# tbuckworth/train-procgen-pytorch

Hardware: AMD Instinct MI355X
Metric: env steps/sec (whole node), coinrun hard-500 IMPALA-CNN PPO (higher is better)
Workload: dtype bf16

## Files before the change

### train-procgen-pytorch_amd/csrc/device_util.h

```cpp
#pragma once
#include <hip/hip_runtime.h>
#include <stdint.h>

typedef short bf16x8 __attribute__((ext_vector_type(8)));
typedef short s16x4 __attribute__((ext_vector_type(4)));
typedef s16x4 __attribute__((address_space(3))) * lds_s16x4_ptr;
#define MFMA16(a, b, c) __builtin_amdgcn_mfma_f32_16x16x4f32((a), (b), (c), 0, 0, 0)
#define MFMA_BF16(a, b, c) __builtin_amdgcn_mfma_f32_16x16x32_bf16((a), (b), (c), 0, 0, 0)

template <typename T>
__device__ __forceinline__ T wave_sum(T v) {
#pragma unroll
    for (int o = 32; o > 0; o >>= 1) v += __shfl_down(v, o, 64);
    return v;
}
__device__ __forceinline__ float wave_max(float v) {
#pragma unroll
    for (int o = 32; o > 0; o >>= 1) v = fmaxf(v, __shfl_down(v, o, 64));
    return v;
}
template <typename T>
__device__ __forceinline__ T block_sum256(T v, T* sbuf) {
    v = wave_sum(v);
    const int lane = threadIdx.x & 63, w = threadIdx.x >> 6;
// ... 48 lines not shown
#pragma unroll
    for (int j = 0; j < 2; ++j)
        lo[j] = __builtin_amdgcn_perm(__builtin_amdgcn_perm((unsigned)best[4 * j + 3], (unsigned)best[4 * j + 2], 0x0c0c0400u),
                                      __builtin_amdgcn_perm((unsigned)best[4 * j + 1], (unsigned)best[4 * j], 0x0c0c0400u), 0x05040100u);
    val = (uint4){mi_keys_to_bf16x2(kv[0]), mi_keys_to_bf16x2(kv[1]), mi_keys_to_bf16x2(kv[2]), mi_keys_to_bf16x2(kv[3])};
    arg = (uint2){0x08080808u - lo[0], 0x08080808u - lo[1]};
}
__device__ __forceinline__ unsigned mi_relu_bf16x2(unsigned w) {
    return __builtin_bit_cast(unsigned, __builtin_elementwise_max(__builtin_bit_cast(mi_s16x2, w), (mi_s16x2){0, 0}));
}
__device__ __forceinline__ float mi_bf16x4_lane(uint2 w, int r) {
    const unsigned u = (r >> 1) ? w.y : w.x;
    return (r & 1) ? bfw_hi(u) : bfw_lo(u);
}
__device__ __forceinline__ uint2 mi_pk_bf16x4(const float (&v)[4]) { return (uint2){mi_pk_bf16(v[0], v[1]), mi_pk_bf16(v[2], v[3])}; }
```

### train-procgen-pytorch_amd/csrc/resblock_bf16.hip

```cpp
#include "common.h"
#include "device_util.h"
#include <hip/hip_ext.h>
#include <mutex>
#include <type_traits>

__device__ __forceinline__ bool rb_pos(uint2 w, int r) {
    const unsigned u = (r >> 1) ? w.y : w.x;
    return (r & 1) ? (int)u >= 0x10000 : (short)(unsigned short)u > (short)0;
}

#ifndef RB_ROWPAD8
#define RB_ROWPAD8 1
#endif
#ifndef RB_SWZ16
#define RB_SWZ16 1
#endif
#ifndef RB_S32
#define RB_S32 48
#endif
template <int C_, int HW_, int TH_, int NIMG_, int NT_ = 256>
struct RbCfg {
    static constexpr int C = C_, HW = HW_, TH = TH_, NIMG = NIMG_, NT = NT_, NW = NT_ / 64;
    static constexpr bool WHOLE = (TH == HW);
    static_assert(WHOLE || NIMG == 1, "row tiles hold one image");
// ... 384 lines not shown
    static constexpr size_t LDS_BYTES = (size_t)5 * T_ELEMS * 2;
    static_assert(LDS_BYTES <= 160 * 1024 && NMT % 8 == 0 && NPX * 4 % 256 == 0, "one workgroup per CU; tile pairs per wave; whole staging words");
    static __device__ __forceinline__ int org(int pl) { return (pl / (HW * HW)) * IMG_ELEMS + (((pl / HW) % HW) * P + pl % HW) * S; }
};
template <class C>
__global__ __launch_bounds__(512, 2) void resblock_pair32r_bf16_kernel(ResblockPairArgs a) {
    extern __shared__ __attribute__((aligned(16))) unsigned short smem_h[];
    unsigned short* s_x = smem_h;
    unsigned short* s_a1 = s_x + C::T_ELEMS;
    unsigned short* s_h = s_a1 + C::T_ELEMS;
    unsigned short* s_a2 = s_h + 2 * C::T_ELEMS;
    const int tid = threadIdx.x, lane = tid & 63, i = lane & 15, kq = lane >> 4;
    const int wv = __builtin_amdgcn_readfirstlane(tid >> 6);
    const bool role_a = wv < 4;
    const int rw = wv & 3;
    for (int e = tid; e < 5 * C::T_ELEMS / 8; e += 512) ((uint4*)smem_h)[e] = (uint4){0u, 0u, 0u, 0u};
    f32x4 st[36];
    f32x4 bq[2][2];
    {
        const unsigned short* bk1 = a.bank[role_a ? 0 : 2];
        const unsigned short* bk2 = a.bank[role_a ? 1 : 3];
        const float* b1 = a.b[role_a ? 0 : 2];
        const float* b2 = a.b[role_a ? 1 : 3];
#pragma unroll
        for (int m = 0; m < 9; ++m)
#pragma unroll
            for (int nb = 0; nb < 2; ++nb) {
                st[2 * m + nb] = __builtin_bit_cast(f32x4, *(const uint4*)(bk1 + (nb * 16 + i) * C::WS + m * 32 + kq * 8));
                st[18 + 2 * m + nb] = __builtin_bit_cast(f32x4, *(const uint4*)(bk2 + (nb * 16 + i) * C::WS + m * 32 + kq * 8));
            }
#pragma unroll
        for (int nb = 0; nb < 2; ++nb) { bq[0][nb] = *(const f32x4*)(b1 + nb * 16 + kq * 4); bq[1][nb] = *(const f32x4*)(b2 + nb * 16 + kq * 4); }
    }
    __builtin_amdgcn_s_waitcnt(0x0F70);
    auto koffc = [](int m) { return ((m / 3) * C::P + (m % 3)) * C::S; };
    constexpr int CENTER = (C::P + 1) * C::S;
    const int nitem = (a.n + C::NIMG - 1) / C::NIMG;
    const int nimg = ((int)blockIdx.x < nitem) ? (nitem - 1 - (int)blockIdx.x) / (int)gridDim.x + 1 : 0;
    typedef unsigned rp_u32x4 __attribute__((ext_vector_type(4)));
    rp_u32x4 rx[C::NWORD];
    auto load = [&](int k) {
        const long long it = blockIdx.x + (long long)(k < nimg ? k : nimg - 1) * gridDim.x;
#pragma unroll
        for (int q = 0; q < C::NWORD; ++q) {
            if constexpr (C::NIMG == 1) rx[q] = *(const rp_u32x4*)(a.x + it * (C::HW * C::HW * C::C) + (size_t)(tid + q * 256) * 8);
            else {
                const int e = tid + q * 256, pl = e >> 2;
                long long n = it * C::NIMG + pl / (C::HW * C::HW); n = n < a.n ? n : a.n - 1;
                rx[q] = *(const rp_u32x4*)(a.x + (n * (C::HW * C::HW) + pl % (C::HW * C::HW)) * C::C + (e & 3) * 8);
            }
        }
    };
    auto conv_tiles = [&](const unsigned short* s_src, const int (&org)[2], const int b0, bool relu, f32x4 (&acc)[2][2]) {
        bf16x8 av[2][5];
        auto rd = [&](int q, int m) {
            bf16x8 v = *(const bf16x8*)(s_src + org[q] + kq * 8 + koffc(m));
            if (relu) { const uint4 u = __builtin_bit_cast(uint4, v); v = __builtin_bit_cast(bf16x8, (uint4){mi_relu_bf16x2(u.x), mi_relu_bf16x2(u.y), mi_relu_bf16x2(u.z), mi_relu_bf16x2(u.w)}); }
            return v;
        };
#pragma unroll
// ... 15 lines not shown
    if (role_a && nimg > 0) load(0);
    for (int step = 0; step <= nimg; ++step) {
        const bool on = role_a ? step < nimg : step >= 1;
        const int k = role_a ? step : step - 1;
        const long long item0 = (blockIdx.x + (long long)(k < 0 ? 0 : k) * gridDim.x) * C::NIMG;
        const long long base = item0 * (C::HW * C::HW * C::C);
        const int left = a.n - (int)item0;
        unsigned short* s_in = role_a ? s_x : s_h + ((step - 1) & 1) * C::T_ELEMS;
        unsigned short* s_mid = role_a ? s_a1 : s_a2;
        unsigned short* a_out = role_a ? a.a1_out : a.a2_out;
        unsigned short* y_out = role_a ? a.y1_out : a.y2_out;
        __syncthreads();
        if (role_a && on) {
#pragma unroll
            for (int q = 0; q < C::NWORD; ++q) {
                const int e = tid + q * 256, pl = e >> 2;
                *(rp_u32x4*)(s_x + C::org(pl) + CENTER + (e & 3) * 8) = rx[q];
            }
            load(step + 1);
        }
        __syncthreads();
        if (on) {
            for (int t = rw; t < C::NMT; t += 8) {
                int pl[2], org[2];
#pragma unroll
                for (int q2 = 0; q2 < 2; ++q2) { pl[q2] = (t + 4 * q2) * 16 + i; org[q2] = C::org(pl[q2]); }
                f32x4 acc[2][2];
                conv_tiles(s_in, org, 0, true, acc);
#pragma unroll
                for (int q2 = 0; q2 < 2; ++q2)
#pragma unroll
                    for (int nb = 0; nb < 2; ++nb) {
                        float v[4];
#pragma unroll
                        for (int r = 0; r < 4; ++r) v[r] = acc[q2][nb][r] + bq[0][nb][r];
                        const uint2 raw = mi_pk_bf16x4(v);
                        if (a_out && (C::NIMG == 1 || pl[q2] / (C::HW * C::HW) < left)) *(uint2*)(a_out + base + (long long)pl[q2] * C::C + nb * 16 + kq * 4) = raw;
                        *(uint2*)(s_mid + org[q2] + CENTER + nb * 16 + kq * 4) = (uint2){mi_relu_bf16x2(raw.x), mi_relu_bf16x2(raw.y)};
                    }
            }
        }
        __syncthreads();
        if (on) {
            unsigned short* s_nxt = s_h + (step & 1) * C::T_ELEMS;
            for (int t = rw; t < C::NMT; t += 8) {
                int pl[2], org[2];
                uint2 sk[2][2];
#pragma unroll
                for (int q2 = 0; q2 < 2; ++q2) {
                    pl[q2] = (t + 4 * q2) * 16 + i; org[q2] = C::org(pl[q2]);
                    sk[q2][0] = *(const uint2*)(s_in + org[q2] + CENTER + kq * 4); sk[q2][1] = *(const uint2*)(s_in + org[q2] + CENTER + 16 + kq * 4);
                }
                f32x4 acc[2][2];
                conv_tiles(s_mid, org, 18, false, acc);
#pragma unroll
                for (int q2 = 0; q2 < 2; ++q2)
#pragma unroll
                    for (int nb = 0; nb < 2; ++nb) {
                        float v[4];
#pragma unroll
                        for (int r = 0; r < 4; ++r) v[r] = acc[q2][nb][r] + bq[1][nb][r] + mi_bf16x4_lane(sk[q2][nb], r);
                        const uint2 raw = mi_pk_bf16x4(v);
                        if (y_out && (C::NIMG == 1 || pl[q2] / (C::HW * C::HW) < left)) *(uint2*)(y_out + base + (long long)pl[q2] * C::C + nb * 16 + kq * 4) = raw;
                        if (role_a) *(uint2*)(s_nxt + org[q2] + CENTER + nb * 16 + kq * 4) = raw;
                    }
            }
        }
    }
}
template <class C>
static void launch_rbp32r(const ResblockPairArgs& a, hipStream_t st) {
    static std::once_flag attr;
    std::call_once(attr, [] { hipFuncSetAttribute((const void*)resblock_pair32r_bf16_kernel<C>, hipFuncAttributeMaxDynamicSharedMemorySize, (int)C::LDS_BYTES); });
    const int items = (a.n + C::NIMG - 1) / C::NIMG, grid = items > 256 ? 256 : items;
    if (grid < 1) return;
    hipLaunchKernelGGL(resblock_pair32r_bf16_kernel<C>, dim3(grid), dim3(512), C::LDS_BYTES, st, a);
}
using RBR_32_16 = RbPair32R<16, 1>;

template <class C>
// ... 289 lines not shown
                                   const unsigned short* bank2_t, const unsigned short* bank1_t, float* slab2, float* slab1, hipStream_t st, hipEvent_t done_ev) {
    const int grid = resblock_bwd_full_grid(n);
    if (grid < 1) return;
    RbFullArgs a{(const unsigned short*)dy, (const unsigned short*)a_fwd, (const unsigned short*)x_fwd, (unsigned short*)dx_out, (unsigned short*)da_out,
                 bank2_t, bank1_t, slab2, slab1, n};
    constexpr size_t LDS_D = RBFULL16D_NBUF * RbFull16S::TILE_BYTES > RbFull16S::RED_BYTES ? RBFULL16D_NBUF * RbFull16S::TILE_BYTES : RbFull16S::RED_BYTES;
    static_assert(LDS_D > 80 * 1024 && LDS_D <= 160 * 1024, "one workgroup per CU");
    static std::once_flag attr;
    std::call_once(attr, [] { hipFuncSetAttribute((const void*)resblock_bwd_full16d_bf16_kernel, hipFuncAttributeMaxDynamicSharedMemorySize, (int)LDS_D); });
    if (done_ev) hipExtLaunchKernelGGL(resblock_bwd_full16d_bf16_kernel, dim3(grid), dim3(512), (unsigned)LDS_D, st, nullptr, done_ev, 0, a);
    else hipLaunchKernelGGL(resblock_bwd_full16d_bf16_kernel, dim3(grid), dim3(512), LDS_D, st, a);
}

template <int HW_, int NT_, int TH_>
struct RbFull32T {
    static constexpr int C = 32, HW = HW_, TH = TH_, S = RB_S32, P = HW + 2, TPI = HW / TH, NT = NT_;
    static constexpr int XR = TH + 4, YR = TH + 2;
    static constexpr int X_ELEMS = XR * P * S, Y_ELEMS = YR * P * S;
    static constexpr int NK = 9, WS = NK * 32 + 16;
    static constexpr int NMT1 = YR * HW / 16, NMT2 = TH * HW / 16;
    static constexpr int NX = XR * HW * 4, NA = YR * HW * 4;
    static constexpr int NSTEP = TH * HW / 32;
    static constexpr int NQ = 18;
    static constexpr int WLEN = C * 9 * C, SLAB = WLEN + C;
};
#ifndef RB32S_TH
#define RB32S_TH 16
#endif
using RbFull32W = RbFull32T<16, 512, RB32S_TH>;
#ifdef WG_TIMING
__device__ unsigned long long g_rb_timing[8];
#define RTCK(k) do { if ((tid & 255) == 0) { const long long now_ = clock64(); tacc_[k] += now_ - tlast_; tlast_ = now_; } } while (0)
#else
#define RTCK(k) do { } while (0)
#endif
template <class C>
__global__ __launch_bounds__(512, 2) void resblock_bwd_full32s_bf16_kernel(RbFullArgs a) {
    static_assert(C::NT == 512 && C::HW == 16, "16x16 images, 8 waves");
    extern __shared__ __attribute__((aligned(16))) unsigned short smem_h[];
    unsigned short* s_x = smem_h;
    unsigned short* s_y = s_x + C::X_ELEMS;
    unsigned short* s_a = s_y + C::Y_ELEMS;
    unsigned short* s_p = s_a + C::Y_ELEMS;
    const int tid = threadIdx.x, lane = tid & 63, wave = tid >> 6, i = lane & 15, kq = lane >> 4, rq = (lane & 15) >> 2, cp = lane & 3;
    const int wv = __builtin_amdgcn_readfirstlane(wave);
    const bool conv_role = wv < 4;
#ifdef WG_TIMING
    long long tacc_[4] = {0, 0, 0, 0}, tlast_ = clock64();
#endif
    const int rw = wv & 3;
    for (int e = tid; e < (C::X_ELEMS + 3 * C::Y_ELEMS) / 8; e += C::NT) ((uint4*)smem_h)[e] = (uint4){0u, 0u, 0u, 0u};
    constexpr bool WHOLE = C::TPI == 1;
    constexpr int NT2 = 256, NIN = C::HW * C::HW * 4;
    constexpr int KX2 = WHOLE ? NIN / NT2 : (C::NX + NT2 - 1) / NT2, KA2 = WHOLE ? NIN / NT2 : (C::NA + NT2 - 1) / NT2;
    static_assert(!WHOLE || NIN % NT2 == 0, "whole words per staging thread");
    constexpr int NST = (22 + KX2 + 2 * KA2) > 36 ? (22 + KX2 + 2 * KA2) : 36;
    f32x4 st[NST];
    constexpr int QM = 5;
    const int qcnt = (C::NQ - rw + 3) / 4;
    if (conv_role) {
#pragma unroll
        for (int m = 0; m < 9; ++m)
#pragma unroll
            for (int nb = 0; nb < 2; ++nb) {
                st[2 * m + nb] = __builtin_bit_cast(f32x4, *(const uint4*)(a.bank2_t + (nb * 16 + i) * C::WS + m * 32 + kq * 8));
                st[18 + 2 * m + nb] = __builtin_bit_cast(f32x4, *(const uint4*)(a.bank1_t + (nb * 16 + i) * C::WS + m * 32 + kq * 8));
            }
    } else {
#pragma unroll
        for (int q = 0; q < NST; ++q) st[q] = (f32x4){0.f, 0.f, 0.f, 0.f};
    }
    __builtin_amdgcn_s_waitcnt(0x0F70);
    const bf16x8 ones = __builtin_bit_cast(bf16x8, (uint4){0x3f803f80u, 0x3f803f80u, 0x3f803f80u, 0x3f803f80u});
    auto koffc = [](int m) { return ((m / 3) * C::P + (m % 3)) * C::S; };

    const int nwork = a.n * C::TPI;
    const int t2 = tid - 256;
    auto load = [&](int work) {
        const long long img = work / C::TPI; const int ty0 = (work % C::TPI) * C::TH;
        if constexpr (WHOLE) {
            const long long o = img * (C::HW * C::HW * C::C) + t2 * 8;
#pragma unroll
            for (int k = 0; k < KX2; ++k) {
                st[22 + k] = __builtin_bit_cast(f32x4, *(const uint4*)(a.dy + o + k * NT2 * 8));
                st[22 + KX2 + k] = __builtin_bit_cast(f32x4, *(const uint4*)(a.a_fwd + o + k * NT2 * 8));
                st[22 + KX2 + KA2 + k] = __builtin_bit_cast(f32x4, *(const uint4*)(a.x_fwd + o + k * NT2 * 8));
            }
            return;
        }
#pragma unroll
        for (int k = 0; k < KX2; ++k) {
            const int e = t2 + k * NT2;
            uint4 v = {0u, 0u, 0u, 0u};
            if (e < C::NX) { const int c8 = e & 3, px = (e >> 2) % C::HW, gy = ty0 - 2 + e / (4 * C::HW);
                             if (gy >= 0 && gy < C::HW) v = *(const uint4*)(a.dy + ((img * C::HW + gy) * C::HW + px) * C::C + c8 * 8); }
            st[22 + k] = __builtin_bit_cast(f32x4, v);
        }
#pragma unroll
        for (int k = 0; k < KA2; ++k) {
            const int e = t2 + k * NT2;
            uint4 va = {0u, 0u, 0u, 0u}, vp = {0u, 0u, 0u, 0u};
            if (e < C::NA) { const int c8 = e & 3, px = (e >> 2) % C::HW, gy = ty0 - 1 + e / (4 * C::HW);
                             if (gy >= 0 && gy < C::HW) { const long long o = ((img * C::HW + gy) * C::HW + px) * C::C + c8 * 8;
                                                          va = *(const uint4*)(a.a_fwd + o); vp = *(const uint4*)(a.x_fwd + o); } }
            st[22 + KX2 + k] = __builtin_bit_cast(f32x4, va); st[22 + KX2 + KA2 + k] = __builtin_bit_cast(f32x4, vp);
        }
    };
    const int orow0 = ((kq >> 1) * C::P + 4 * (kq & 1) + rq) * C::S + 4 * cp;
    struct WgBase { int d, b[QM]; };
    auto wg_bases = [&](const unsigned short* s_d, int d_off, const unsigned short* s_src) {
        WgBase w;
        w.d = (int)(s_d - smem_h) + orow0 + d_off;
#pragma unroll
        for (int qq = 0; qq < QM; ++qq) {
            const int q = rw + 4 * (qq < 4 ? qq : (qcnt > 4 ? 4 : 0)), tap = q >> 1, ib = q & 1;
            w.b[qq] = (int)(s_src - smem_h) + orow0 + ((tap / 3) * C::P + (tap % 3)) * C::S + ib * 16;
            asm volatile("" : "+v"(w.b[qq]));
        }
        asm volatile("" : "+v"(w.d));
        return w;
// ... 10 lines not shown
        for (int cb = 0; cb < 2; ++cb) d[cb] = tr(w.d, cb * 16);
#pragma unroll
        for (int qq = 0; qq < QM; ++qq) b[qq] = tr(w.b[qq], 0);
        asm volatile("" ::: "memory");
        if (bias) { st[20] = MFMA_BF16(d[0], ones, st[20]); st[21] = MFMA_BF16(d[1], ones, st[21]); }
#pragma unroll
        for (int qq = 0; qq < QM; ++qq)
            if (qq < qcnt) {
#pragma unroll
                for (int cb = 0; cb < 2; ++cb) st[a0 + 2 * qq + cb] = MFMA_BF16(d[cb], b[qq], st[a0 + 2 * qq + cb]);
            }
    };

    if (!conv_role && (int)blockIdx.x < nwork) load(blockIdx.x);
    for (int work = blockIdx.x; work < nwork; work += gridDim.x) {
        const long long img = work / C::TPI; const int ty0 = (work % C::TPI) * C::TH;
        __syncthreads();
        RTCK(3);
        if (!conv_role && WHOLE) {
            const int o = ((t2 >> 6) * C::P + ((t2 >> 2) & (C::HW - 1)) + 1) * C::S + (t2 & 3) * 8;
#pragma unroll
            for (int k = 0; k < KX2; ++k) {
                const int ok = o + k * (NT2 / 64) * C::P * C::S;
                const uint4 va = __builtin_bit_cast(uint4, st[22 + KX2 + k]), vp = __builtin_bit_cast(uint4, st[22 + KX2 + KA2 + k]);
                *(uint4*)(s_x + ok + 2 * C::P * C::S) = __builtin_bit_cast(uint4, st[22 + k]);
                *(uint4*)(s_a + ok + C::P * C::S) = (uint4){mi_relu_bf16x2(va.x), mi_relu_bf16x2(va.y), mi_relu_bf16x2(va.z), mi_relu_bf16x2(va.w)};
                *(uint4*)(s_p + ok + C::P * C::S) = (uint4){mi_relu_bf16x2(vp.x), mi_relu_bf16x2(vp.y), mi_relu_bf16x2(vp.z), mi_relu_bf16x2(vp.w)};
            }
        } else if (!conv_role) {
#pragma unroll
            for (int k = 0; k < KX2; ++k) {
                const int e = t2 + k * NT2;
                if (e < C::NX) *(uint4*)(s_x + ((e / (4 * C::HW)) * C::P + (e >> 2) % C::HW + 1) * C::S + (e & 3) * 8) = __builtin_bit_cast(uint4, st[22 + k]);
            }
#pragma unroll
            for (int k = 0; k < KA2; ++k) {
                const int e = t2 + k * NT2;
                if (e < C::NA) {
                    const int o = ((e / (4 * C::HW)) * C::P + (e >> 2) % C::HW + 1) * C::S + (e & 3) * 8;
                    const uint4 va = __builtin_bit_cast(uint4, st[22 + KX2 + k]), vp = __builtin_bit_cast(uint4, st[22 + KX2 + KA2 + k]);
                    *(uint4*)(s_a + o) = (uint4){mi_relu_bf16x2(va.x), mi_relu_bf16x2(va.y), mi_relu_bf16x2(va.z), mi_relu_bf16x2(va.w)};
                    *(uint4*)(s_p + o) = (uint4){mi_relu_bf16x2(vp.x), mi_relu_bf16x2(vp.y), mi_relu_bf16x2(vp.z), mi_relu_bf16x2(vp.w)};
                }
            }
        }
        __syncthreads();
        RTCK(0);
        if (!conv_role && work + (int)gridDim.x < nwork) load(work + gridDim.x);

        if (conv_role) {
            for (int t = rw; t < C::NMT1; t += 4) {
                const int pl = t * 16 + i, px = pl % C::HW, ry = pl / C::HW;
                const unsigned short* src = s_x + (ry * C::P + px) * C::S + kq * 8;
                const int yb = (ry * C::P + px + 1) * C::S + kq * 4;
                bf16x8 av[5];
#pragma unroll
                for (int m = 0; m < 5; ++m) av[m] = *(const bf16x8*)(src + koffc(m));
                const uint2 mk0 = *(const uint2*)(s_a + yb), mk1 = *(const uint2*)(s_a + yb + 16);
                asm volatile("" ::: "memory");
                f32x4 acc[2] = {{0.f, 0.f, 0.f, 0.f}, {0.f, 0.f, 0.f, 0.f}};
#pragma unroll
                for (int m = 0; m < 9; ++m) {
                    const bf16x8 cur = av[m % 5];
                    acc[0] = MFMA_BF16(__builtin_bit_cast(bf16x8, st[2 * m]), cur, acc[0]);
                    acc[1] = MFMA_BF16(__builtin_bit_cast(bf16x8, st[2 * m + 1]), cur, acc[1]);
                    if (m < 4) av[m] = *(const bf16x8*)(src + koffc(m + 5));
                }
#pragma unroll
                for (int nb = 0; nb < 2; ++nb) {
                    const uint2 mk = nb ? mk1 : mk0;
                    float v[4];
#pragma unroll
                    for (int r = 0; r < 4; ++r) v[r] = rb_pos(mk, r) ? acc[nb][r] : 0.f;
                    const uint2 raw = mi_pk_bf16x4(v);
                    *(uint2*)(s_y + yb + nb * 16) = raw;
                    if (a.da_out) {
                        const int gy = ty0 - 1 + ry;
                        if (ry >= 1 && ry <= C::TH) *(uint2*)(a.da_out + ((img * C::HW + gy) * C::HW + px) * C::C + nb * 16 + kq * 4) = raw;
                    }
                }
            }
        } else {
            const WgBase wb = wg_bases(s_x, (2 * C::P + 1) * C::S, s_a);
#pragma unroll
            for (int t = 0; t < C::NSTEP; ++t) wg_step(t, wb, 0, rw == 2);
        }
        RTCK(1);
        __syncthreads();
        RTCK(2);
        if (conv_role) {
            for (int t = rw; t < C::NMT2; t += 4) {
                const int pl = t * 16 + i, px = pl % C::HW, oy = pl / C::HW;
                const unsigned short* src = s_y + (oy * C::P + px) * C::S + kq * 8;
                bf16x8 av[5];
#pragma unroll
                for (int m = 0; m < 5; ++m) av[m] = *(const bf16x8*)(src + koffc(m));
                const int eo = ((oy + 1) * C::P + px + 1) * C::S + kq * 4;
                const uint2 mk0 = *(const uint2*)(s_p + eo), mk1 = *(const uint2*)(s_p + eo + 16);
                const uint2 sk0 = *(const uint2*)(s_x + eo + C::P * C::S), sk1 = *(const uint2*)(s_x + eo + C::P * C::S + 16);
                asm volatile("" ::: "memory");
                f32x4 acc[2] = {{0.f, 0.f, 0.f, 0.f}, {0.f, 0.f, 0.f, 0.f}};
#pragma unroll
                for (int m = 0; m < 9; ++m) {
                    const bf16x8 cur = av[m % 5];
                    acc[0] = MFMA_BF16(__builtin_bit_cast(bf16x8, st[18 + 2 * m]), cur, acc[0]);
                    acc[1] = MFMA_BF16(__builtin_bit_cast(bf16x8, st[18 + 2 * m + 1]), cur, acc[1]);
                    if (m < 4) av[m] = *(const bf16x8*)(src + koffc(m + 5));
                }
#pragma unroll
                for (int nb = 0; nb < 2; ++nb) {
                    const uint2 mk = nb ? mk1 : mk0, sk = nb ? sk1 : sk0;
                    float v[4];
#pragma unroll
                    for (int r = 0; r < 4; ++r) v[r] = (rb_pos(mk, r) ? acc[nb][r] : 0.f) + mi_bf16x4_lane(sk, r);
                    *(uint2*)(a.dx_out + ((img * C::HW + ty0 + oy) * C::HW + px) * C::C + nb * 16 + kq * 4) = mi_pk_bf16x4(v);
                }
            }
        } else {
            const WgBase wb = wg_bases(s_y, (C::P + 1) * C::S, s_p);
#pragma unroll
            for (int t = 0; t < C::NSTEP; ++t) wg_step(t, wb, 10, rw == 3);
        }
    }
#ifdef WG_TIMING
    if ((tid & 255) == 0) for (int q = 0; q < 4; ++q) atomicAdd(&g_rb_timing[(tid >> 8) * 4 + q], (unsigned long long)tacc_[q]);
#endif
    if (!conv_role) {
        float* sl2 = a.slab2 + (long long)blockIdx.x * C::SLAB;
        float* sl1 = a.slab1 + (long long)blockIdx.x * C::SLAB;
#pragma unroll
        for (int qq = 0; qq < QM; ++qq)
// ... 27 lines not shown
    static constexpr int NQ = 18, WLEN = C * 9 * C, SLAB = WLEN + C;
    static constexpr size_t LDS_BYTES = (size_t)4 * T_ELEMS * 2;
    static_assert(LDS_BYTES <= 160 * 1024, "one workgroup per CU");
};
__global__ __launch_bounds__(512, 2) void resblock_bwd_full32q_bf16_kernel(RbFullArgs a) {
    using C = RbFull32Q;
    extern __shared__ __attribute__((aligned(16))) unsigned short smem_h[];
    unsigned short* s_x = smem_h;
    unsigned short* s_y = s_x + C::T_ELEMS;
    unsigned short* s_a = s_y + C::T_ELEMS;
    unsigned short* s_p = s_a + C::T_ELEMS;
    const int tid = threadIdx.x, lane = tid & 63, wave = tid >> 6, i = lane & 15, kq = lane >> 4, rq = (lane & 15) >> 2, cp = lane & 3;
    const int wv = __builtin_amdgcn_readfirstlane(wave);
    const bool conv_role = wv < 4;
    const int rw = wv & 3;
#ifdef WG_TIMING
    long long tacc_[4] = {0, 0, 0, 0}, tlast_ = clock64();
#endif
    for (int e = tid; e < 4 * C::T_ELEMS / 8; e += 512) ((uint4*)smem_h)[e] = (uint4){0u, 0u, 0u, 0u};
    constexpr int NST = 36, QM = 5;
    static_assert(22 + 3 * C::KW <= NST, "prefetch words fit behind the accumulators");
    f32x4 st[NST];
    const int qcnt = (C::NQ - rw + 3) / 4;
    if (conv_role) {
#pragma unroll
        for (int m = 0; m < 9; ++m)
#pragma unroll
            for (int nb = 0; nb < 2; ++nb) {
                st[2 * m + nb] = __builtin_bit_cast(f32x4, *(const uint4*)(a.bank2_t + (nb * 16 + i) * C::WS + m * 32 + kq * 8));
                st[18 + 2 * m + nb] = __builtin_bit_cast(f32x4, *(const uint4*)(a.bank1_t + (nb * 16 + i) * C::WS + m * 32 + kq * 8));
// ... 87 lines not shown
                const unsigned short* src = s_x + org + kq * 8;
                const int yb = org + CENTER + kq * 4;
                bf16x8 av[5];
#pragma unroll
                for (int m = 0; m < 5; ++m) av[m] = *(const bf16x8*)(src + koffc(m));
                const uint2 mk0 = *(const uint2*)(s_a + yb), mk1 = *(const uint2*)(s_a + yb + 16);
                asm volatile("" ::: "memory");
                f32x4 acc[2] = {{0.f, 0.f, 0.f, 0.f}, {0.f, 0.f, 0.f, 0.f}};
#pragma unroll
                for (int m = 0; m < 9; ++m) {
                    const bf16x8 cur = av[m % 5];
                    acc[0] = MFMA_BF16(__builtin_bit_cast(bf16x8, st[2 * m]), cur, acc[0]);
                    acc[1] = MFMA_BF16(__builtin_bit_cast(bf16x8, st[2 * m + 1]), cur, acc[1]);
                    if (m < 4) av[m] = *(const bf16x8*)(src + koffc(m + 5));
                }
#pragma unroll
                for (int nb = 0; nb < 2; ++nb) {
                    const uint2 mk = nb ? mk1 : mk0;
                    float v[4];
#pragma unroll
                    for (int r = 0; r < 4; ++r) v[r] = rb_pos(mk, r) ? acc[nb][r] : 0.f;
                    const uint2 raw = mi_pk_bf16x4(v);
                    *(uint2*)(s_y + yb + nb * 16) = raw;
                    if (a.da_out) {
                        const int pl = t * 16 + i;
                        if ((pl >> 6) < left) *(uint2*)(a.da_out + ((long long)img0 * 64 + pl) * C::C + nb * 16 + kq * 4) = raw;
                    }
                }
            }
        } else {
            const WgBase wb = wg_bases(s_x, s_a);
#pragma unroll
            for (int t = 0; t < C::NSTEP; ++t) wg_step(t, wb, 0, rw == 2);
        }
        RTCK(1);
        __syncthreads();
        RTCK(2);
        if (conv_role) {
            for (int t = rw; t < C::NMT; t += 4) {
                const int pl = t * 16 + i, org = porg(pl);
                const unsigned short* src = s_y + org + kq * 8;
                const int eo = org + CENTER + kq * 4;
                bf16x8 av[5];
#pragma unroll
                for (int m = 0; m < 5; ++m) av[m] = *(const bf16x8*)(src + koffc(m));
                const uint2 mk0 = *(const uint2*)(s_p + eo), mk1 = *(const uint2*)(s_p + eo + 16);
                const uint2 sk0 = *(const uint2*)(s_x + eo), sk1 = *(const uint2*)(s_x + eo + 16);
                asm volatile("" ::: "memory");
                f32x4 acc[2] = {{0.f, 0.f, 0.f, 0.f}, {0.f, 0.f, 0.f, 0.f}};
#pragma unroll
                for (int m = 0; m < 9; ++m) {
                    const bf16x8 cur = av[m % 5];
                    acc[0] = MFMA_BF16(__builtin_bit_cast(bf16x8, st[18 + 2 * m]), cur, acc[0]);
                    acc[1] = MFMA_BF16(__builtin_bit_cast(bf16x8, st[18 + 2 * m + 1]), cur, acc[1]);
                    if (m < 4) av[m] = *(const bf16x8*)(src + koffc(m + 5));
                }
                if ((pl >> 6) < left) {
#pragma unroll
                    for (int nb = 0; nb < 2; ++nb) {
                        const uint2 mk = nb ? mk1 : mk0, sk = nb ? sk1 : sk0;
                        float v[4];
#pragma unroll
                        for (int r = 0; r < 4; ++r) v[r] = (rb_pos(mk, r) ? acc[nb][r] : 0.f) + mi_bf16x4_lane(sk, r);
                        *(uint2*)(a.dx_out + ((long long)img0 * 64 + pl) * C::C + nb * 16 + kq * 4) = mi_pk_bf16x4(v);
                    }
                }
            }
        } else {
            const WgBase wb = wg_bases(s_y, s_p);
#pragma unroll
            for (int t = 0; t < C::NSTEP; ++t) wg_step(t, wb, 10, rw == 3);
        }
    }
#ifdef WG_TIMING
    if ((tid & 255) == 0) for (int q = 0; q < 4; ++q) atomicAdd(&g_rb_timing[(tid >> 8) * 4 + q], (unsigned long long)tacc_[q]);
#endif
    if (!conv_role) {
        float* sl2 = a.slab2 + (long long)blockIdx.x * C::SLAB;
        float* sl1 = a.slab1 + (long long)blockIdx.x * C::SLAB;
#pragma unroll
        for (int qq = 0; qq < QM; ++qq)
// ... 13 lines not shown
            for (int cb = 0; cb < 2; ++cb)
#pragma unroll
                for (int r = 0; r < 4; ++r) sl[C::WLEN + cb * 16 + kq * 4 + r] = st[20 + cb][r];
        }
    }
}
static int rb_full32q_grid(int n) { const int w = (n + RbFull32Q::NIMG - 1) / RbFull32Q::NIMG; return w > 256 ? 256 : w; }
static void launch_rb_full32q(const RbFullArgs& a, hipStream_t st) {
    static std::once_flag attr;
    std::call_once(attr, [] { hipFuncSetAttribute((const void*)resblock_bwd_full32q_bf16_kernel, hipFuncAttributeMaxDynamicSharedMemorySize, (int)RbFull32Q::LDS_BYTES); });
    const int grid = rb_full32q_grid(a.n);
    if (grid < 1) return;
    hipLaunchKernelGGL(resblock_bwd_full32q_bf16_kernel, dim3(grid), dim3(512), RbFull32Q::LDS_BYTES, st, a);
}

static int rb_full32s_grid(int n) { const int w = n * RbFull32W::TPI; return w > 256 ? 256 : w; }
static void launch_rb_full32s(const RbFullArgs& a, hipStream_t st) {
    using C = RbFull32W;
    constexpr size_t LDS = (size_t)(C::X_ELEMS + 3 * C::Y_ELEMS) * 2;
    static std::once_flag attr;
    std::call_once(attr, [] { hipFuncSetAttribute((const void*)resblock_bwd_full32s_bf16_kernel<C>, hipFuncAttributeMaxDynamicSharedMemorySize, (int)LDS); });
    const int grid = rb_full32s_grid(a.n);
    if (grid < 1) return;
    hipLaunchKernelGGL(resblock_bwd_full32s_bf16_kernel<C>, dim3(grid), dim3(512), LDS, st, a);
}
int resblock_bwd_full32_grid(ConvShape s, int n) { return s == CS_32_32_16 ? rb_full32s_grid(n) : s == CS_32_32_8 ? rb_full32q_grid(n) : -1; }
void launch_resblock_bwd_full32_bf16(ConvShape s, const void* dy, const void* a_fwd, const void* x_fwd, void* dx_out, void* da_out, int n,
                                     const unsigned short* bank2_t, const unsigned short* bank1_t, float* slab2, float* slab1, hipStream_t st) {
    RbFullArgs a{(const unsigned short*)dy, (const unsigned short*)a_fwd, (const unsigned short*)x_fwd, (unsigned short*)dx_out, (unsigned short*)da_out,
                 bank2_t, bank1_t, slab2, slab1, n};
    if (s == CS_32_32_16) launch_rb_full32s(a, st);
// ... 15 lines not shown
```

Measured before the change: 725,700.

## Widen resblock epilogue stores to 16-byte words via permlane16 swap

Epilogue outputs of the fused resblock forward and backward kernels are repacked across lane halves with permlane16_swap, so each lane writes one 16-byte chunk to LDS and global memory instead of two 8-byte words. This is meant to cut LDS bank conflicts and store instruction count. The full32s backward kernel also drops its row-tile path so phase 1 covers only the 16 interior rows, and the staging address math is simplified. It adds cross-lane permutes and relies on the new chunk layout matching what later reads expect. A scratch Python bank-conflict model is included.

```diff
diff --git a/scratch/lds_bank_model.py b/scratch/lds_bank_model.py
--- /dev/null
+++ b/scratch/lds_bank_model.py
@@ -0,0 +1,141 @@
+
+S_BYTES, P, HW = 96, 18, 16
+_G128 = [list(range(0, 4)) + list(range(12, 16)) + list(range(20, 28)), list(range(4, 12)) + list(range(16, 20)) + list(range(28, 32))]
+INSTR = {
+    "ds_read_b64": (8, 64, [list(range(0, 32)), list(range(32, 64))]),
+    "ds_read_b64_tr_b16": (8, 64, [list(range(0, 32)), list(range(32, 64))]),
+    "ds_read_b128": (16, 64, _G128 + [[l + 32 for l in g] for g in _G128]),
+    "ds_write_b64": (8, 32, [list(range(16 * g, 16 * g + 16)) for g in range(4)]),
+    "ds_write_b128": (16, 32, [list(range(8 * g, 8 * g + 8)) for g in range(8)]),
+}
+
+
+def cycles(instr, addr):
+    nbytes, banks, groups = INSTR[instr]
+    assert len(addr) == 64 and all(a % min(nbytes, 16) == 0 for a in addr), "one aligned address per lane"
+    total = 0
+    for g in groups:
+        per_bank = {}
+        for lane in g:
+            for d in range(addr[lane] // 4, (addr[lane] + nbytes) // 4):
+                per_bank.setdefault(d % banks, set()).add(d)
+        total += max(len(v) for v in per_bank.values())
+    return total
+
+
+def free_cycles(instr):
+    return len(INSTR[instr][2])
+
+
+def pix(row, col):
+    return (row * P + col) * S_BYTES
+
+
+def _lane(l):
+    return l & 15, l >> 4
+
+
+
+def operand_read(t, tap):
+    return [pix(t + tap // 3, _lane(l)[0] + tap % 3) + 16 * _lane(l)[1] for l in range(64)]
+
+
+def epilogue_store(t, wide, nb=0):
+    if wide:
+        return [pix(t + 1, _lane(l)[0] + 1) + (_lane(l)[1] & 1) * 32 + (_lane(l)[1] >> 1) * 16 for l in range(64)]
+    return [pix(t + 1, _lane(l)[0] + 1) + nb * 32 + _lane(l)[1] * 8 for l in range(64)]
+
+
+def mask_read(t, nb, wide=False):
+    return epilogue_store(t, True) if wide else epilogue_store(t, False, nb)
+
+
+def transposing_read(step, second, col_bytes=0, tap=4):
+    out = []
+    for l in range(64):
+        kq, rq, cp = l >> 4, (l & 15) >> 2, l & 3
+        out.append(pix(2 * step + (kq >> 1) + tap // 3, 4 * (kq & 1) + rq + 8 * second + tap % 3) + col_bytes + 8 * cp)
+    return out
+
+
+def staging_store(wave, k):
+    return [pix((64 * wave + l + 256 * k) // 64 + 1, ((64 * wave + l) >> 2) % HW + 1) + 16 * (l & 3) for l in range(64)]
+
+
+def chunk_swizzle(addr, fn):
+    out = []
+    for a in addr:
+        p, off = divmod(a, S_BYTES)
+        out.append(p * S_BYTES + 16 * fn(off // 16, p % P) + off % 16)
+    return out
+
+
+
+def store_cycles(t, wide):
+    return cycles("ds_write_b128", epilogue_store(t, True)) if wide else sum(cycles("ds_write_b64", epilogue_store(t, False, nb)) for nb in (0, 1))
+
+
+def conv_tile(t, wide, stores=True, reads=1):
+    c = sum(cycles("ds_read_b128", operand_read(t, tap)) for tap in range(9))
+    c += reads * sum(cycles("ds_read_b64", mask_read(t, nb)) for nb in (0, 1))
+    return c + (store_cycles(t, wide) if stores else 0)
+
+
+def staging(tensors):
+    return tensors * sum(cycles("ds_write_b128", staging_store(w, k)) for w in range(4) for k in range(4))
+
+
+def pair32r_image(wide):
+    c = 2 * sum(conv_tile(t, wide, reads=0) for t in range(HW))
+    c += sum(conv_tile(t, wide) for t in range(HW)) + sum(conv_tile(t, wide, stores=False) for t in range(HW))
+    return c + staging(1)
+
+
+def full32s_image(wide, tiles1=HW + 2):
+    c = sum(conv_tile(t % HW, wide) for t in range(tiles1)) + sum(conv_tile(t, wide, stores=False, reads=2) for t in range(HW)) + staging(3)
+    free = tiles1 * (36 + 2 * free_cycles("ds_read_b64") + (free_cycles("ds_write_b128") if wide else 2 * free_cycles("ds_write_b64")))
+    free += HW * (36 + 4 * free_cycles("ds_read_b64")) + 3 * 16 * free_cycles("ds_write_b128")
+    wg = 2 * 4 * sum(cycles("ds_read_b64_tr_b16", transposing_read(s, h)) for s in range(HW // 2) for h in (0, 1)) * 7
+    return c + wg, c - free
+
+
+def swizzle_survey():
+    fns = {"none": lambda c, x: c}
+    for bit in (2, 3):
+        for m in (1, 2, 3):
+            fns[f"xor {m} on column bit {bit}"] = lambda c, x, m=m, bit=bit: c ^ (m * ((x >> bit) & 1)) if c < 4 else c
+        for r in (1, 2, 3):
+            fns[f"rotate {r} of 6 on column bit {bit}"] = lambda c, x, r=r, bit=bit: (c + r * ((x >> bit) & 1)) % 6
+    out = []
+    for name, fn in fns.items():
+        st = sum(cycles("ds_write_b64", chunk_swizzle(epilogue_store(3, False, nb), fn)) for nb in (0, 1))
+        rd = max(cycles("ds_read_b128", chunk_swizzle(operand_read(3, tap), fn)) for tap in range(9))
+        out.append((name, st, rd))
+    return out
+
+
+def main():
+    print("array cycles per wave-instruction (conflict-free count in brackets)")
+    rows = [("operand read, worst tap", "ds_read_b128", max(cycles("ds_read_b128", operand_read(3, tap)) for tap in range(9))),
+            ("epilogue store, 8-byte word", "ds_write_b64", cycles("ds_write_b64", epilogue_store(3, False))),
+            ("epilogue store, 16-byte chunk", "ds_write_b128", cycles("ds_write_b128", epilogue_store(3, True))),
+            ("mask / skip read, 8-byte word", "ds_read_b64", cycles("ds_read_b64", mask_read(3, 0))),
+            ("mask / skip read, 16-byte chunk", "ds_read_b128", cycles("ds_read_b128", mask_read(3, 0, True))),
+            ("transposing read", "ds_read_b64_tr_b16", cycles("ds_read_b64_tr_b16", transposing_read(1, 0))),
+            ("staging store", "ds_write_b128", cycles("ds_write_b128", staging_store(0, 0)))]
+    for what, ins, c in rows:
+        print(f"  {what:34s} {ins:20s} {c:3d}  [{free_cycles(ins)}]")
+    print("per pixel tile: stores before %d, after %d; full32s phase-1 tile before %d, after %d" % (
+        store_cycles(3, False), store_cycles(3, True), conv_tile(3, False), conv_tile(3, True)))
+    b, a = pair32r_image(False), pair32r_image(True)
+    print("pair32r per image: before %d, after %d (%+.1f %%)" % (b, a, 100.0 * (a - b) / b))
+    (b, bc), (w, wc), (a, ac) = full32s_image(False), full32s_image(True), full32s_image(True, HW)
+    print("full32s per image: before %d (%.1f %% conflict cycles), wide stores %d (%.1f %%), wide stores and 16 phase-1 tiles %d (%.1f %%)" % (
+        b, 100.0 * bc / b, w, 100.0 * wc / w, a, 100.0 * ac / a))
+    print("swizzles (8-byte stores of a tile; worst operand read):")
+    for name, st, rd in swizzle_survey():
+        print(f"  {name:34s} stores {st:3d}   operand read {rd}")
+
+
+if __name__ == "__main__":
+    main()
diff --git a/train-procgen-pytorch_amd/csrc/device_util.h b/train-procgen-pytorch_amd/csrc/device_util.h
--- a/train-procgen-pytorch_amd/csrc/device_util.h
+++ b/train-procgen-pytorch_amd/csrc/device_util.h
@@ -86,3 +86,12 @@
     return (r & 1) ? bfw_hi(u) : bfw_lo(u);
 }
 __device__ __forceinline__ uint2 mi_pk_bf16x4(const float (&v)[4]) { return (uint2){mi_pk_bf16(v[0], v[1]), mi_pk_bf16(v[2], v[3])}; }
+
+__device__ __forceinline__ uint4 mi_wide32_word(uint2 w0, uint2 w1) {
+    const auto x = __builtin_amdgcn_permlane16_swap(w0.x, w1.x, false, false);
+    const auto y = __builtin_amdgcn_permlane16_swap(w0.y, w1.y, false, false);
+    return (uint4){x[0], y[0], x[1], y[1]};
+}
+__device__ __forceinline__ int mi_wide32_byte_off(int kq) { return (kq & 1) * 32 + (kq >> 1) * 16; }
+__device__ __forceinline__ int mi_wide32_off(int kq) { return mi_wide32_byte_off(kq) / 2; }
+__device__ __forceinline__ uint4 mi_relu_bf16x8(uint4 w) { return (uint4){mi_relu_bf16x2(w.x), mi_relu_bf16x2(w.y), mi_relu_bf16x2(w.z), mi_relu_bf16x2(w.w)}; }
diff --git a/train-procgen-pytorch_amd/csrc/resblock_bf16.hip b/train-procgen-pytorch_amd/csrc/resblock_bf16.hip
--- a/train-procgen-pytorch_amd/csrc/resblock_bf16.hip
+++ b/train-procgen-pytorch_amd/csrc/resblock_bf16.hip
@@ -422,6 +422,7 @@
     const int wv = __builtin_amdgcn_readfirstlane(tid >> 6);
     const bool role_a = wv < 4;
     const int rw = wv & 3;
+    const int wq = mi_wide32_off(kq);
     for (int e = tid; e < 5 * C::T_ELEMS / 8; e += 512) ((uint4*)smem_h)[e] = (uint4){0u, 0u, 0u, 0u};
     f32x4 st[36];
     f32x4 bq[2][2];
@@ -451,7 +452,7 @@
         const long long it = blockIdx.x + (long long)(k < nimg ? k : nimg - 1) * gridDim.x;
 #pragma unroll
         for (int q = 0; q < C::NWORD; ++q) {
-            if constexpr (C::NIMG == 1) rx[q] = *(const rp_u32x4*)(a.x + it * (C::HW * C::HW * C::C) + (size_t)(tid + q * 256) * 8);
+            if constexpr (C::NIMG == 1) rx[q] = *(const rp_u32x4*)((const char*)(a.x + it * (C::HW * C::HW * C::C) + q * 256 * 8) + (unsigned)tid * 16u);
             else {
                 const int e = tid + q * 256, pl = e >> 2;
                 long long n = it * C::NIMG + pl / (C::HW * C::HW); n = n < a.n ? n : a.n - 1;
@@ -497,8 +498,12 @@
         if (role_a && on) {
 #pragma unroll
             for (int q = 0; q < C::NWORD; ++q) {
-                const int e = tid + q * 256, pl = e >> 2;
-                *(rp_u32x4*)(s_x + C::org(pl) + CENTER + (e & 3) * 8) = rx[q];
+                if constexpr (C::NIMG == 1 && 64 % C::HW == 0) {
+                    *(rp_u32x4*)(s_x + C::org(tid >> 2) + CENTER + (tid & 3) * 8 + q * (64 / C::HW) * C::P * C::S) = rx[q];
+                } else {
+                    const int e = tid + q * 256, pl = e >> 2;
+                    *(rp_u32x4*)(s_x + C::org(pl) + CENTER + (e & 3) * 8) = rx[q];
+                }
             }
             load(step + 1);
         }
@@ -511,16 +516,19 @@
                 f32x4 acc[2][2];
                 conv_tiles(s_in, org, 0, true, acc);
 #pragma unroll
-                for (int q2 = 0; q2 < 2; ++q2)
+                for (int q2 = 0; q2 < 2; ++q2) {
+                    uint2 raw[2];
 #pragma unroll
                     for (int nb = 0; nb < 2; ++nb) {
                         float v[4];
 #pragma unroll
                         for (int r = 0; r < 4; ++r) v[r] = acc[q2][nb][r] + bq[0][nb][r];
-                        const uint2 raw = mi_pk_bf16x4(v);
-                        if (a_out && (C::NIMG == 1 || pl[q2] / (C::HW * C::HW) < left)) *(uint2*)(a_out + base + (long long)pl[q2] * C::C + nb * 16 + kq * 4) = raw;
-                        *(uint2*)(s_mid + org[q2] + CENTER + nb * 16 + kq * 4) = (uint2){mi_relu_bf16x2(raw.x), mi_relu_bf16x2(raw.y)};
+                        raw[nb] = mi_pk_bf16x4(v);
                     }
+                    const uint4 w = mi_wide32_word(raw[0], raw[1]);
+                    if (a_out && (C::NIMG == 1 || pl[q2] / (C::HW * C::HW) < left)) *(uint4*)((char*)(a_out + base) + (unsigned)(pl[q2] * C::C + wq) * 2u) = w;
+                    *(uint4*)(s_mid + org[q2] + CENTER + wq) = mi_relu_bf16x8(w);
+                }
             }
         }
         __syncthreads();
@@ -537,16 +545,19 @@
                 f32x4 acc[2][2];
                 conv_tiles(s_mid, org, 18, false, acc);
 #pragma unroll
-                for (int q2 = 0; q2 < 2; ++q2)
+                for (int q2 = 0; q2 < 2; ++q2) {
+                    uint2 raw[2];
 #pragma unroll
                     for (int nb = 0; nb < 2; ++nb) {
                         float v[4];
 #pragma unroll
                         for (int r = 0; r < 4; ++r) v[r] = acc[q2][nb][r] + bq[1][nb][r] + mi_bf16x4_lane(sk[q2][nb], r);
-                        const uint2 raw = mi_pk_bf16x4(v);
-                        if (y_out && (C::NIMG == 1 || pl[q2] / (C::HW * C::HW) < left)) *(uint2*)(y_out + base + (long long)pl[q2] * C::C + nb * 16 + kq * 4) = raw;
-                        if (role_a) *(uint2*)(s_nxt + org[q2] + CENTER + nb * 16 + kq * 4) = raw;
+                        raw[nb] = mi_pk_bf16x4(v);
                     }
+                    const uint4 w = mi_wide32_word(raw[0], raw[1]);
+                    if (y_out && (C::NIMG == 1 || pl[q2] / (C::HW * C::HW) < left)) *(uint4*)((char*)(y_out + base) + (unsigned)(pl[q2] * C::C + wq) * 2u) = w;
+                    if (role_a) *(uint4*)(s_nxt + org[q2] + CENTER + wq) = w;
+                }
             }
         }
     }
@@ -866,20 +877,17 @@
 
 template <int HW_, int NT_, int TH_>
 struct RbFull32T {
-    static constexpr int C = 32, HW = HW_, TH = TH_, S = RB_S32, P = HW + 2, TPI = HW / TH, NT = NT_;
+    static_assert(TH_ == HW_, "whole-image items");
+    static constexpr int C = 32, HW = HW_, TH = TH_, S = RB_S32, P = HW + 2, NT = NT_;
     static constexpr int XR = TH + 4, YR = TH + 2;
     static constexpr int X_ELEMS = XR * P * S, Y_ELEMS = YR * P * S;
     static constexpr int NK = 9, WS = NK * 32 + 16;
-    static constexpr int NMT1 = YR * HW / 16, NMT2 = TH * HW / 16;
-    static constexpr int NX = XR * HW * 4, NA = YR * HW * 4;
+    static constexpr int NMT = TH * HW / 16;
     static constexpr int NSTEP = TH * HW / 32;
     static constexpr int NQ = 18;
     static constexpr int WLEN = C * 9 * C, SLAB = WLEN + C;
 };
-#ifndef RB32S_TH
-#define RB32S_TH 16
-#endif
-using RbFull32W = RbFull32T<16, 512, RB32S_TH>;
+using RbFull32W = RbFull32T<16, 512, 16>;
 #ifdef WG_TIMING
 __device__ unsigned long long g_rb_timing[8];
 #define RTCK(k) do { if ((tid & 255) == 0) { const long long now_ = clock64(); tacc_[k] += now_ - tlast_; tlast_ = now_; } } while (0)
@@ -901,11 +909,11 @@
     long long tacc_[4] = {0, 0, 0, 0}, tlast_ = clock64();
 #endif
     const int rw = wv & 3;
+    const int wq = mi_wide32_off(kq);
     for (int e = tid; e < (C::X_ELEMS + 3 * C::Y_ELEMS) / 8; e += C::NT) ((uint4*)smem_h)[e] = (uint4){0u, 0u, 0u, 0u};
-    constexpr bool WHOLE = C::TPI == 1;
     constexpr int NT2 = 256, NIN = C::HW * C::HW * 4;
-    constexpr int KX2 = WHOLE ? NIN / NT2 : (C::NX + NT2 - 1) / NT2, KA2 = WHOLE ? NIN / NT2 : (C::NA + NT2 - 1) / NT2;
-    static_assert(!WHOLE || NIN % NT2 == 0, "whole words per staging thread");
+    constexpr int KX2 = NIN / NT2, KA2 = NIN / NT2;
+    static_assert(NIN % NT2 == 0, "whole words per staging thread");
     constexpr int NST = (22 + KX2 + 2 * KA2) > 36 ? (22 + KX2 + 2 * KA2) : 36;
     f32x4 st[NST];
     constexpr int QM = 5;
@@ -926,36 +934,15 @@
     const bf16x8 ones = __builtin_bit_cast(bf16x8, (uint4){0x3f803f80u, 0x3f803f80u, 0x3f803f80u, 0x3f803f80u});
     auto koffc = [](int m) { return ((m / 3) * C::P + (m % 3)) * C::S; };
 
-    const int nwork = a.n * C::TPI;
+    const int nwork = a.n;
     const int t2 = tid - 256;
     auto load = [&](int work) {
-        const long long img = work / C::TPI; const int ty0 = (work % C::TPI) * C::TH;
-        if constexpr (WHOLE) {
-            const long long o = img * (C::HW * C::HW * C::C) + t2 * 8;
-#pragma unroll
-            for (int k = 0; k < KX2; ++k) {
-                st[22 + k] = __builtin_bit_cast(f32x4, *(const uint4*)(a.dy + o + k * NT2 * 8));
-                st[22 + KX2 + k] = __builtin_bit_cast(f32x4, *(const uint4*)(a.a_fwd + o + k * NT2 * 8));
-                st[22 + KX2 + KA2 + k] = __builtin_bit_cast(f32x4, *(const uint4*)(a.x_fwd + o + k * NT2 * 8));
-            }
-            return;
-        }
+        const long long o = (long long)work * (C::HW * C::HW * C::C) + t2 * 8;
 #pragma unroll
         for (int k = 0; k < KX2; ++k) {
-            const int e = t2 + k * NT2;
-            uint4 v = {0u, 0u, 0u, 0u};
-            if (e < C::NX) { const int c8 = e & 3, px = (e >> 2) % C::HW, gy = ty0 - 2 + e / (4 * C::HW);
-                             if (gy >= 0 && gy < C::HW) v = *(const uint4*)(a.dy + ((img * C::HW + gy) * C::HW + px) * C::C + c8 * 8); }
-            st[22 + k] = __builtin_bit_cast(f32x4, v);
-        }
-#pragma unroll
-        for (int k = 0; k < KA2; ++k) {
-            const int e = t2 + k * NT2;
-            uint4 va = {0u, 0u, 0u, 0u}, vp = {0u, 0u, 0u, 0u};
-            if (e < C::NA) { const int c8 = e & 3, px = (e >> 2) % C::HW, gy = ty0 - 1 + e / (4 * C::HW);
-                             if (gy >= 0 && gy < C::HW) { const long long o = ((img * C::HW + gy) * C::HW + px) * C::C + c8 * 8;
-                                                          va = *(const uint4*)(a.a_fwd + o); vp = *(const uint4*)(a.x_fwd + o); } }
-            st[22 + KX2 + k] = __builtin_bit_cast(f32x4, va); st[22 + KX2 + KA2 + k] = __builtin_bit_cast(f32x4, vp);
+            st[22 + k] = __builtin_bit_cast(f32x4, *(const uint4*)(a.dy + o + k * NT2 * 8));
+            st[22 + KX2 + k] = __builtin_bit_cast(f32x4, *(const uint4*)(a.a_fwd + o + k * NT2 * 8));
+            st[22 + KX2 + KA2 + k] = __builtin_bit_cast(f32x4, *(const uint4*)(a.x_fwd + o + k * NT2 * 8));
         }
     };
     const int orow0 = ((kq >> 1) * C::P + 4 * (kq & 1) + rq) * C::S + 4 * cp;
@@ -996,10 +983,10 @@
 
     if (!conv_role && (int)blockIdx.x < nwork) load(blockIdx.x);
     for (int work = blockIdx.x; work < nwork; work += gridDim.x) {
-        const long long img = work / C::TPI; const int ty0 = (work % C::TPI) * C::TH;
+        const long long img = work;
         __syncthreads();
         RTCK(3);
-        if (!conv_role && WHOLE) {
+        if (!conv_role) {
             const int o = ((t2 >> 6) * C::P + ((t2 >> 2) & (C::HW - 1)) + 1) * C::S + (t2 & 3) * 8;
 #pragma unroll
             for (int k = 0; k < KX2; ++k) {
@@ -1009,30 +996,14 @@
                 *(uint4*)(s_a + ok + C::P * C::S) = (uint4){mi_relu_bf16x2(va.x), mi_relu_bf16x2(va.y), mi_relu_bf16x2(va.z), mi_relu_bf16x2(va.w)};
                 *(uint4*)(s_p + ok + C::P * C::S) = (uint4){mi_relu_bf16x2(vp.x), mi_relu_bf16x2(vp.y), mi_relu_bf16x2(vp.z), mi_relu_bf16x2(vp.w)};
             }
-        } else if (!conv_role) {
-#pragma unroll
-            for (int k = 0; k < KX2; ++k) {
-                const int e = t2 + k * NT2;
-                if (e < C::NX) *(uint4*)(s_x + ((e / (4 * C::HW)) * C::P + (e >> 2) % C::HW + 1) * C::S + (e & 3) * 8) = __builtin_bit_cast(uint4, st[22 + k]);
-            }
-#pragma unroll
-            for (int k = 0; k < KA2; ++k) {
-                const int e = t2 + k * NT2;
-                if (e < C::NA) {
-                    const int o = ((e / (4 * C::HW)) * C::P + (e >> 2) % C::HW + 1) * C::S + (e & 3) * 8;
-                    const uint4 va = __builtin_bit_cast(uint4, st[22 + KX2 + k]), vp = __builtin_bit_cast(uint4, st[22 + KX2 + KA2 + k]);
-                    *(uint4*)(s_a + o) = (uint4){mi_relu_bf16x2(va.x), mi_relu_bf16x2(va.y), mi_relu_bf16x2(va.z), mi_relu_bf16x2(va.w)};
-                    *(uint4*)(s_p + o) = (uint4){mi_relu_bf16x2(vp.x), mi_relu_bf16x2(vp.y), mi_relu_bf16x2(vp.z), mi_relu_bf16x2(vp.w)};
-                }
-            }
         }
         __syncthreads();
         RTCK(0);
         if (!conv_role && work + (int)gridDim.x < nwork) load(work + gridDim.x);
 
         if (conv_role) {
-            for (int t = rw; t < C::NMT1; t += 4) {
-                const int pl = t * 16 + i, px = pl % C::HW, ry = pl / C::HW;
+            for (int t = rw; t < C::NMT; t += 4) {
+                const int pl = t * 16 + i, px = pl % C::HW, ry = pl / C::HW + 1;
                 const unsigned short* src = s_x + (ry * C::P + px) * C::S + kq * 8;
                 const int yb = (ry * C::P + px + 1) * C::S + kq * 4;
                 bf16x8 av[5];
@@ -1048,19 +1019,18 @@
                     acc[1] = MFMA_BF16(__builtin_bit_cast(bf16x8, st[2 * m + 1]), cur, acc[1]);
                     if (m < 4) av[m] = *(const bf16x8*)(src + koffc(m + 5));
                 }
+                uint2 raw[2];
 #pragma unroll
                 for (int nb = 0; nb < 2; ++nb) {
                     const uint2 mk = nb ? mk1 : mk0;
                     float v[4];
 #pragma unroll
                     for (int r = 0; r < 4; ++r) v[r] = rb_pos(mk, r) ? acc[nb][r] : 0.f;
-                    const uint2 raw = mi_pk_bf16x4(v);
-                    *(uint2*)(s_y + yb + nb * 16) = raw;
-                    if (a.da_out) {
-                        const int gy = ty0 - 1 + ry;
-                        if (ry >= 1 && ry <= C::TH) *(uint2*)(a.da_out + ((img * C::HW + gy) * C::HW + px) * C::C + nb * 16 + kq * 4) = raw;
-                    }
-                }
+                    raw[nb] = mi_pk_bf16x4(v);
+                }
+                const uint4 w = mi_wide32_word(raw[0], raw[1]);
+                *(uint4*)(s_y + yb - kq * 4 + wq) = w;
+                if (a.da_out) *(uint4*)(a.da_out + (img * (C::HW * C::HW) + pl) * C::C + wq) = w;
             }
         } else {
             const WgBase wb = wg_bases(s_x, (2 * C::P + 1) * C::S, s_a);
@@ -1071,7 +1041,7 @@
         __syncthreads();
         RTCK(2);
         if (conv_role) {
-            for (int t = rw; t < C::NMT2; t += 4) {
+            for (int t = rw; t < C::NMT; t += 4) {
                 const int pl = t * 16 + i, px = pl % C::HW, oy = pl / C::HW;
                 const unsigned short* src = s_y + (oy * C::P + px) * C::S + kq * 8;
                 bf16x8 av[5];
@@ -1089,14 +1059,16 @@
                     acc[1] = MFMA_BF16(__builtin_bit_cast(bf16x8, st[18 + 2 * m + 1]), cur, acc[1]);
                     if (m < 4) av[m] = *(const bf16x8*)(src + koffc(m + 5));
                 }
+                uint2 raw[2];
 #pragma unroll
                 for (int nb = 0; nb < 2; ++nb) {
                     const uint2 mk = nb ? mk1 : mk0, sk = nb ? sk1 : sk0;
                     float v[4];
 #pragma unroll
                     for (int r = 0; r < 4; ++r) v[r] = (rb_pos(mk, r) ? acc[nb][r] : 0.f) + mi_bf16x4_lane(sk, r);
-                    *(uint2*)(a.dx_out + ((img * C::HW + ty0 + oy) * C::HW + px) * C::C + nb * 16 + kq * 4) = mi_pk_bf16x4(v);
-                }
+                    raw[nb] = mi_pk_bf16x4(v);
+                }
+                *(uint4*)(a.dx_out + (img * (C::HW * C::HW) + pl) * C::C + wq) = mi_wide32_word(raw[0], raw[1]);
             }
         } else {
             const WgBase wb = wg_bases(s_y, (C::P + 1) * C::S, s_p);
@@ -1154,6 +1126,7 @@
     const int wv = __builtin_amdgcn_readfirstlane(wave);
     const bool conv_role = wv < 4;
     const int rw = wv & 3;
+    const int wq = mi_wide32_off(kq);
 #ifdef WG_TIMING
     long long tacc_[4] = {0, 0, 0, 0}, tlast_ = clock64();
 #endif
@@ -1271,18 +1244,20 @@
                     acc[1] = MFMA_BF16(__builtin_bit_cast(bf16x8, st[2 * m + 1]), cur, acc[1]);
                     if (m < 4) av[m] = *(const bf16x8*)(src + koffc(m + 5));
                 }
+                uint2 raw[2];
 #pragma unroll
                 for (int nb = 0; nb < 2; ++nb) {
                     const uint2 mk = nb ? mk1 : mk0;
                     float v[4];
 #pragma unroll
                     for (int r = 0; r < 4; ++r) v[r] = rb_pos(mk, r) ? acc[nb][r] : 0.f;
-                    const uint2 raw = mi_pk_bf16x4(v);
-                    *(uint2*)(s_y + yb + nb * 16) = raw;
-                    if (a.da_out) {
-                        const int pl = t * 16 + i;
-                        if ((pl >> 6) < left) *(uint2*)(a.da_out + ((long long)img0 * 64 + pl) * C::C + nb * 16 + kq * 4) = raw;
-                    }
+                    raw[nb] = mi_pk_bf16x4(v);
+                }
+                const uint4 w = mi_wide32_word(raw[0], raw[1]);
+                *(uint4*)(s_y + yb - kq * 4 + wq) = w;
+                if (a.da_out) {
+                    const int pl = t * 16 + i;
+                    if ((pl >> 6) < left) *(uint4*)(a.da_out + ((long long)img0 * 64 + pl) * C::C + wq) = w;
                 }
             }
         } else {
@@ -1312,16 +1287,17 @@
                     acc[1] = MFMA_BF16(__builtin_bit_cast(bf16x8, st[18 + 2 * m + 1]), cur, acc[1]);
                     if (m < 4) av[m] = *(const bf16x8*)(src + koffc(m + 5));
                 }
-                if ((pl >> 6) < left) {
-#pragma unroll
-                    for (int nb = 0; nb < 2; ++nb) {
-                        const uint2 mk = nb ? mk1 : mk0, sk = nb ? sk1 : sk0;
-                        float v[4];
-#pragma unroll
-                        for (int r = 0; r < 4; ++r) v[r] = (rb_pos(mk, r) ? acc[nb][r] : 0.f) + mi_bf16x4_lane(sk, r);
-                        *(uint2*)(a.dx_out + ((long long)img0 * 64 + pl) * C::C + nb * 16 + kq * 4) = mi_pk_bf16x4(v);
-                    }
-                }
+                uint2 raw[2];
+#pragma unroll
+                for (int nb = 0; nb < 2; ++nb) {
+                    const uint2 mk = nb ? mk1 : mk0, sk = nb ? sk1 : sk0;
+                    float v[4];
+#pragma unroll
+                    for (int r = 0; r < 4; ++r) v[r] = (rb_pos(mk, r) ? acc[nb][r] : 0.f) + mi_bf16x4_lane(sk, r);
+                    raw[nb] = mi_pk_bf16x4(v);
+                }
+                const uint4 w = mi_wide32_word(raw[0], raw[1]);
+                if ((pl >> 6) < left) *(uint4*)(a.dx_out + ((long long)img0 * 64 + pl) * C::C + wq) = w;
             }
         } else {
             const WgBase wb = wg_bases(s_y, s_p);
@@ -1365,7 +1341,7 @@
     hipLaunchKernelGGL(resblock_bwd_full32q_bf16_kernel, dim3(grid), dim3(512), RbFull32Q::LDS_BYTES, st, a);
 }
 
-static int rb_full32s_grid(int n) { const int w = n * RbFull32W::TPI; return w > 256 ? 256 : w; }
+static int rb_full32s_grid(int n) { return n > 256 ? 256 : n; }
 static void launch_rb_full32s(const RbFullArgs& a, hipStream_t st) {
     using C = RbFull32W;
     constexpr size_t LDS = (size_t)(C::X_ELEMS + 3 * C::Y_ELEMS) * 2;
```

New measurement: 729,900, median of 3. No clear change (+0.6%).
